# safes/RayTracing-Weekend

Hardware: AMD Instinct MI355X
Metric: Msamples/s, Cornell box 1920x1080 4096spp (higher is better)
Workload: dtype f32

## Files before the change

raytracing_weekend_amd/csrc/rtw_device.h:

```cpp
#pragma once
#include <hip/hip_runtime.h>
#include <stdint.h>

#include "../../include/rtw.h"

#define RTW_DEV __device__ __forceinline__

#define RTW_MATH_FN RTW_DEV
#include "rtw_math.h"
#include "rtw_scene.h"

#ifndef RTW_SHORT_FORMS
#define RTW_SHORT_FORMS 1
#endif

namespace rtwdev {

struct v3 { float x, y, z; };

RTW_DEV v3 V(float x, float y, float z) { v3 r; r.x = x; r.y = y; r.z = z; return r; }
RTW_DEV v3 vadd(v3 a, v3 b) { return V(a.x + b.x, a.y + b.y, a.z + b.z); }
RTW_DEV v3 vsub(v3 a, v3 b) { return V(a.x - b.x, a.y - b.y, a.z - b.z); }
RTW_DEV v3 vmul(v3 a, v3 b) { return V(a.x * b.x, a.y * b.y, a.z * b.z); }
RTW_DEV v3 vscale(v3 a, float s) { return V(a.x * s, a.y * s, a.z * s); }
RTW_DEV v3 vneg(v3 a) { return V(-a.x, -a.y, -a.z); }
RTW_DEV float fma_(float a, float b, float c) { return __builtin_fmaf(a, b, c); }
RTW_DEV v3 vfma(v3 a, float s, v3 b) { return V(fma_(a.x, s, b.x), fma_(a.y, s, b.y), fma_(a.z, s, b.z)); }
RTW_DEV float dot3(v3 a, v3 b) { return fma_(a.z, b.z, fma_(a.y, b.y, a.x * b.x)); }
RTW_DEV v3 cross3(v3 a, v3 b) {
    return V(fma_(a.y, b.z, -(a.z * b.y)), fma_(a.z, b.x, -(a.x * b.z)), fma_(a.x, b.y, -(a.y * b.x)));
}
struct MathHw {
    static RTW_DEV float rcp(float x) { return __builtin_amdgcn_rcpf(x); }
    static RTW_DEV float rsq(float x) { return __builtin_amdgcn_rsqf(x); }
    static RTW_DEV float fma(float a, float b, float c) { return __builtin_fmaf(a, b, c); }
    static RTW_DEV bool all(bool ok) { return __builtin_amdgcn_ballot_w64(!ok) == 0ull; }
};
RTW_DEV float rcp_(float x) { return RTW_SHORT_FORMS ? rtwmath::rcp<MathHw>(x) : 1.0f / x; }
RTW_DEV float sqrt_(float x) { return RTW_SHORT_FORMS ? rtwmath::sqrt<MathHw>(x) : __builtin_sqrtf(x); }
RTW_DEV float sqrt_inside_(float x) { return RTW_SHORT_FORMS ? rtwmath::sqrt_inside<MathHw>(x) : __builtin_sqrtf(x); }
RTW_DEV v3 normalize3(v3 a) {
    const float s = dot3(a, a);
    const float inv = RTW_SHORT_FORMS ? rtwmath::rcp_sqrt<MathHw>(s) : 1.0f / __builtin_sqrtf(s);
    return vscale(a, inv);
}
RTW_DEV float length3(v3 a) { return sqrt_(dot3(a, a)); }
// ... 228 lines not shown
    }
};

typedef uint32_t u32x4 __attribute__((ext_vector_type(4)));
typedef float f32x4 __attribute__((ext_vector_type(4)));

struct DScene {
    const rtw_prim* __restrict__ prims;
    const rtw_xform* __restrict__ xforms;
    const HitRec* __restrict__ hitrec;
    const rtw_light* __restrict__ lights;
    const u32x4* __restrict__ nodes;
    const u32x4* __restrict__ leaves;
    const u32x4* __restrict__ wnodes;
    const int32_t* __restrict__ order;
    const BruteGroup* __restrict__ groups;
    const BruteRec* __restrict__ recs;
    const rtw_texture* __restrict__ texs;
    const uint32_t* __restrict__ texdata;
    const u32x4* __restrict__ walk;
    int32_t n_prims, n_vol, n_tree, n_lights, sky_light, use_bvh, has_motion, n_groups;
    int32_t n_generic;
    int32_t n_walk_words;
    int32_t n_lds_nodes, stack_depth, has_tex, noise_lds_data;
    int32_t n_lds_leaves, stack_wide;
    int32_t n_nodes;
    int32_t estimator;
    float ray_tmin, probe_eps;
    const rtw_light* __restrict__ clights;
    float bmin[3], bmax[3];
    rtw_camera cam;
    rtw_pdf pdf;
    int32_t cam_type;
};

RTW_DEV bool is_volume(int type) { return type == RTW_PRIM_VOLUME_BOX || type == RTW_PRIM_VOLUME_SPHERE; }

#define RTW_CONST __attribute__((address_space(4)))
template <class T>
RTW_DEV const RTW_CONST T* as_const(const T* p) { return (const RTW_CONST T*)(uint64_t)p; }

RTW_DEV rtw_prim load_prim(const DScene& sc, int i) {
    const RTW_CONST u32x4* q = (const RTW_CONST u32x4*)(uint64_t)(sc.prims + i);
    u32x4 a = q[0], b = q[1], c = q[2], d = q[3];
    rtw_prim r;
    r.type = (int)a.x; r.material = (int)a.y; r.xform = (int)a.z; r.flip = (int)a.w;
    r.p[0] = __uint_as_float(b.x); r.p[1] = __uint_as_float(b.y); r.p[2] = __uint_as_float(b.z); r.p[3] = __uint_as_float(b.w);
    r.p[4] = __uint_as_float(c.x); r.p[5] = __uint_as_float(c.y); r.p[6] = __uint_as_float(c.z); r.p[7] = __uint_as_float(c.w);
    r.p[8] = __uint_as_float(d.x); r.p[9] = __uint_as_float(d.y); r.p[10] = __uint_as_float(d.z); r.p[11] = __uint_as_float(d.w);
    return r;
}
struct M34 { float m[12]; };
RTW_DEV M34 load_m34(const float* p) {
    const RTW_CONST f32x4* q = (const RTW_CONST f32x4*)(uint64_t)p;
    f32x4 a = q[0], b = q[1], c = q[2];
    M34 r;
    r.m[0] = a.x; r.m[1] = a.y; r.m[2] = a.z; r.m[3] = a.w;
    r.m[4] = b.x; r.m[5] = b.y; r.m[6] = b.z; r.m[7] = b.w;
    r.m[8] = c.x; r.m[9] = c.y; r.m[10] = c.z; r.m[11] = c.w;
    return r;
}
RTW_DEV M34 load_xf_m(const DScene& sc, int i) { return load_m34(sc.xforms[i].m); }
RTW_DEV M34 load_xf_inv(const DScene& sc, int i) { return load_m34(sc.xforms[i].inv); }
RTW_DEV int load_i32(const int32_t* p) { return *as_const(p); }
typedef uint32_t u32x8 __attribute__((ext_vector_type(8)));
RTW_DEV BruteGroup load_group(const DScene& sc, int i) {
// ... 433 lines not shown
            RTW_RECT_LOOP(G.n_rx, oo.x, inv.x, oo.y, dd.y, oo.z, dd.z)
            RTW_RECT_LOOP(G.n_ry, oo.y, inv.y, oo.x, dd.x, oo.z, dd.z)
            RTW_RECT_LOOP(G.n_rz, oo.z, inv.z, oo.x, dd.x, oo.y, dd.y)
#undef RTW_RECT_LOOP
        }
        for (int i = 0; i < G.n_sph; i++) {
            const BruteRec Rn = load_rec(sc, ++ri);
            float t = 0.f;
            const bool hit = sphere_roots(oo, dd, V(R.a, R.b, R.c), R.d, tmin, RTW_FLT_MAX, t);
            RTW_TAKE(hit, t, R.prim)
            R = Rn;
        }
    }
#undef RTW_TAKE
    if (!GENERIC || (ANY_HIT && best_prim >= 0)) return;
    for (int k = 0; k < sc.n_generic; k++) {
        const int pi = load_i32(sc.order + sc.n_vol + k);
        const rtw_prim pr = load_prim(sc, pi);
        v3 po, pd, mt;
        object_ray(sc, pr, o, d, ray_time, po, pd, mt);
        float t;
        if (prim_test(pr, po, pd, V(0.f, 0.f, 0.f), tmin, RTW_FLT_MAX, gather_time, g, t)) {
            if (t < best_t || (!ANY_HIT && t == best_t && best_prim >= 0 && !best_is_vol && pi < best_prim)) {
                best_t = t; best_prim = pi; best_is_vol = false;
                if (ANY_HIT) return;
            }
        }
    }
}

struct WalkRec { u32x4 q0, q1; };
RTW_DEV bool in_range(float a, uint32_t lo, uint32_t hi) { return __builtin_amdgcn_fmed3f(a, __uint_as_float(lo), __uint_as_float(hi)) == a; }

template <bool ANY_HIT>
RTW_DEV void walk_lds(const u32x4* __restrict__ w, const int n_groups, const v3 o, const v3 d, const float tmin, const float tmax, float& best_t, int& best_prim) {
    uint32_t key_hi = __float_as_uint(tmax), key_lo = 0u;
    const u32x4* xf = w + 2 * n_groups;
    const u32x4* r = w + 5 * n_groups;
    WalkRec A, B;
    A.q0 = r[0]; A.q1 = r[1];
#define RTW_RECT_TEST(R_, OK_, IK_, OA_, DA_, OB_, DB_)                                              \
    {                                                                                                \
        const float t = (__uint_as_float(R_.q1.x) - (OK_)) * (IK_);                                  \
        const float a = fma_(t, (DA_), (OA_));                                                       \
        const float b = fma_(t, (DB_), (OB_));                                                       \
        const bool hit = (t >= tmin) & in_range(a, R_.q0.x, R_.q0.y) & in_range(b, R_.q0.z, R_.q0.w); \
        if (ANY_HIT) {                                                                               \
            key_lo = (hit & (t < tmax)) ? 1u : key_lo;                                               \
        } else {                                                                                     \
            const unsigned long long key = ((unsigned long long)__float_as_uint(t) << 32) | R_.q1.y; \
            const bool take = hit & (key < (((unsigned long long)key_hi << 32) | key_lo));           \
            key_hi = take ? __float_as_uint(t) : key_hi;                                             \
            key_lo = take ? R_.q1.y : key_lo;                                                        \
        }                                                                                            \
    }
#define RTW_REC_LIST(N_, TEST_)                                                                      \
    {                                                                                                \
        int n_ = (N_);                                                                               \
        for (; n_ >= 2; n_ -= 2) {                                                                   \
            B.q0 = r[2]; B.q1 = r[3];                                                                \
            TEST_(A)                                                                                 \
            A.q0 = r[4]; A.q1 = r[5];                                                                \
            TEST_(B)                                                                                 \
            r += 4;                                                                                  \
        }                                                                                            \
        if (n_ > 0) {                                                                                \
            B.q0 = r[2]; B.q1 = r[3];                                                                \
            TEST_(A)                                                                                 \
            A = B;                                                                                   \
            r += 2;                                                                                  \
        }                                                                                            \
    }
    for (int gi = 0; gi < n_groups; gi++) {
        const u32x4 g0 = w[2 * gi], g1 = w[2 * gi + 1];
        const int g_xform = (int)__builtin_amdgcn_readfirstlane(g0.x);
        const int n_rx = (int)__builtin_amdgcn_readfirstlane(g0.z), n_ry = (int)__builtin_amdgcn_readfirstlane(g0.w);
        const int n_rz = (int)__builtin_amdgcn_readfirstlane(g1.x), n_sph = (int)__builtin_amdgcn_readfirstlane(g1.y);
        v3 oo = o, dd = d;
        if (g_xform != 0) {
            const u32x4 r0 = xf[3 * gi], r1 = xf[3 * gi + 1], r2 = xf[3 * gi + 2];
            float m[12];
            m[0] = __uint_as_float(r0.x); m[1] = __uint_as_float(r0.y); m[2] = __uint_as_float(r0.z); m[3] = __uint_as_float(r0.w);
            m[4] = __uint_as_float(r1.x); m[5] = __uint_as_float(r1.y); m[6] = __uint_as_float(r1.z); m[7] = __uint_as_float(r1.w);
            m[8] = __uint_as_float(r2.x); m[9] = __uint_as_float(r2.y); m[10] = __uint_as_float(r2.z); m[11] = __uint_as_float(r2.w);
            oo = xf_point(m, o);
            dd = xf_vector(m, d);
        }
        if (n_rx + n_ry + n_rz > 0) {
            const v3 inv = recip3(dd);
#define RTW_TEST_X(R_) RTW_RECT_TEST(R_, oo.x, inv.x, oo.y, dd.y, oo.z, dd.z)
#define RTW_TEST_Y(R_) RTW_RECT_TEST(R_, oo.y, inv.y, oo.x, dd.x, oo.z, dd.z)
#define RTW_TEST_Z(R_) RTW_RECT_TEST(R_, oo.z, inv.z, oo.x, dd.x, oo.y, dd.y)
            RTW_REC_LIST(n_rx, RTW_TEST_X)
            RTW_REC_LIST(n_ry, RTW_TEST_Y)
            RTW_REC_LIST(n_rz, RTW_TEST_Z)
#undef RTW_TEST_X
#undef RTW_TEST_Y
#undef RTW_TEST_Z
        }
#define RTW_TEST_SPH(R_)                                                                             \
        {                                                                                            \
            float t = 0.f;                                                                           \
            const bool hit = sphere_roots(oo, dd, V(__uint_as_float(R_.q0.x), __uint_as_float(R_.q0.y), __uint_as_float(R_.q0.z)), \
                                          __uint_as_float(R_.q0.w), tmin, RTW_FLT_MAX, t);           \
            if (ANY_HIT) {                                                                           \
                key_lo = (hit & (t < tmax)) ? 1u : key_lo;                                           \
            } else {                                                                                 \
                const unsigned long long key = ((unsigned long long)__float_as_uint(t) << 32) | R_.q1.y; \
                const bool take = hit & (key < (((unsigned long long)key_hi << 32) | key_lo));       \
                key_hi = take ? __float_as_uint(t) : key_hi;                                         \
// ... 352 lines not shown
```

raytracing_weekend_amd/csrc/rtw_hip.hip:

```cpp
#include <hip/hip_runtime.h>

#include <algorithm>
#include <cmath>
#include <cstdio>
#include <cstdlib>
#include <cstring>
#include <condition_variable>
#include <exception>
#include <mutex>
#include <new>
#include <stdexcept>
#include <string>
#include <thread>
#include <vector>

#include "../../include/rtw.h"
#include "rtw_bvh.h"
#include "rtw_scene.h"
#include "rtw_device.h"
#include "rtw_plan.h"
#include "rtw_kernels.h"
#include "rtw_guides.h"
#include "rtw_adaptive.h"
#ifndef RTW_SPLIT_BUILD
// ... 358 lines not shown
    if (c->d_scene) (void)hipFree(c->d_scene);
    if (c->stream) (void)hipStreamDestroy(c->stream);
    delete c;
    return RTW_OK;
}

int upload_prepared(rtw_ctx* c, const PreparedScene& ps) {
    test_fault("upload");
    HIP_TRY(c, hipSetDevice(c->device));
    HIP_TRY(c, hipStreamSynchronize(c->stream));
    if (c->d_scene) { (void)hipFree(c->d_scene); c->d_scene = nullptr; }
    c->has_scene = false;
    HIP_TRY(c, hipMalloc(&c->d_scene, ps.image.size()));
    HIP_TRY(c, hipMemcpy(c->d_scene, ps.image.data(), ps.image.size(), hipMemcpyHostToDevice));
    const char* d = (const char*)c->d_scene;
    const SceneScalars& v = ps.sc;
    const SceneFacts& f = ps.info.facts;
    DScene sc{};
    sc.prims = (const rtw_prim*)(d + ps.off[ST_PRIMS]);
    sc.xforms = (const rtw_xform*)(d + ps.off[ST_XFORMS]);
    sc.hitrec = (const HitRec*)(d + ps.off[ST_HITREC]);
    sc.lights = (const rtw_light*)(d + ps.off[ST_LIGHTS]);
    sc.clights = (const rtw_light*)(d + ps.off[ST_CLIGHTS]);
    sc.nodes = (const u32x4*)(d + ps.off[ST_NODES]);
    sc.wnodes = (const u32x4*)(d + ps.off[ST_WNODES]);
    sc.leaves = (const u32x4*)(d + ps.off[ST_LEAVES]);
    sc.order = (const int32_t*)(d + ps.off[ST_ORDER]);
    sc.groups = (const BruteGroup*)(d + ps.off[ST_GROUPS]);
    sc.recs = (const BruteRec*)(d + ps.off[ST_RECS]);
    sc.texs = (const rtw_texture*)(d + ps.off[ST_TEXS]);
    sc.texdata = (const uint32_t*)(d + ps.off[ST_TEXDATA]);
    sc.walk = (const u32x4*)(d + ps.off[ST_WALK]);
    sc.n_prims = v.n_prims; sc.n_tree = v.n_tree; sc.n_lights = v.n_lights; sc.sky_light = v.sky_light; sc.has_motion = v.has_motion;
    sc.n_groups = v.n_groups; sc.n_generic = v.n_generic; sc.n_walk_words = v.n_walk_words; sc.n_lds_nodes = v.n_lds_nodes; sc.has_tex = v.has_tex;
    sc.noise_lds_data = v.noise_lds_data; sc.n_lds_leaves = v.n_lds_leaves; sc.cam_type = v.cam_type;
    sc.use_bvh = f.use_bvh ? 1 : 0; sc.n_vol = f.n_vol; sc.stack_depth = f.stack_depth; sc.stack_wide = f.stack_wide ? 1 : 0; sc.n_nodes = (int32_t)f.n_tree_nodes;
    sc.estimator = RTW_EST_REFERENCE; sc.ray_tmin = 1e-6f; sc.probe_eps = 500 * 1.0e-7f;
    for (int a = 0; a < 3; a++) { sc.bmin[a] = v.bmin[a]; sc.bmax[a] = v.bmax[a]; }
    sc.cam = v.cam;
    sc.pdf = v.pdf;
    c->sc = sc;
    c->info = ps.info;
    c->has_scene = true;
    return RTW_OK;
}

int impl_upload_scene(rtw_ctx* c, const void* blob, size_t bytes) {
    if (!c) return RTW_ERR_INVALID_ARG;
    if (!c->kids.empty()) c->has_scene = false;
    PreparedScene ps;
    std::string err;
    const int prc = prepare_scene(blob, bytes, read_tuning(), ps, err);
    if (prc) return fail(c, prc, err);
    if (c->kids.empty()) return upload_prepared(c, ps);
    for (rtw_ctx* k : c->kids) {
        const int rc = upload_prepared(k, ps);
        if (rc) return fail(c, rc, k->err);
    }
    c->has_scene = true;
    return RTW_OK;
}

int check_render_args(rtw_ctx* c, const rtw_params* P) {
    if (!c->has_scene) return fail(c, RTW_ERR_NO_SCENE, "rtw_render before rtw_upload_scene");
    if (!P) return fail(c, RTW_ERR_INVALID_ARG, "null params");
    if (P->width <= 0 || P->height <= 0 || P->spp <= 0 || P->max_depth < 0 || P->row0 < 0 || P->row1 > P->height || P->row0 > P->row1)
        return fail(c, RTW_ERR_INVALID_ARG, "bad render params");
// ... 974 lines not shown
```

raytracing_weekend_amd/csrc/rtw_kernels.h:

```cpp
#pragma once
#include "rtw_device.h"
#include "rtw_plan.h"

namespace rtwk {
using namespace rtwdev;

#ifndef RTW_MIN_WAVES
#define RTW_MIN_WAVES 1
#endif
#ifdef RTW_SUBPHASE_TIMERS
constexpr int kSubRows = 16, kSubWaves = 8192;
__device__ unsigned long long g_sub_cyc[kSubWaves][kSubRows];
RTW_DEV constexpr int rtw_sub_id(const char* n) {
    return n[0] != 's' || n[1] != 'a' ? 0 : n[3] == 'h' ? 1 : n[3] == 'l' && n[4] == 'a' ? 2 : n[3] == 'l' ? 3 : n[3] == 'm' ? 4 : n[3] == 'd' ? 5 : n[3] == 'i' ? 6 : n[3] == 'n' ? 7 : 0;
}
RTW_DEV void rtw_sub_stamp(int id) {
    const unsigned long long t_in = __builtin_amdgcn_s_memtime();
    if ((threadIdx.x & 63u) == 0u) {
        unsigned long long* row = g_sub_cyc[(blockIdx.x * (blockDim.x >> 6) + (threadIdx.x >> 6)) % kSubWaves];
        const unsigned long long open_id = row[14], t0 = row[15];
        if (t0 != 0ull) row[open_id] += t_in - t0;
        row[14] = (unsigned long long)id;
        __builtin_amdgcn_s_waitcnt(0);
        row[15] = __builtin_amdgcn_s_memtime();
// ... 1045 lines not shown
                bool alive = false;
                uint32_t nee_prev = (p.gk & kNeePrev) ? 1u : 0u;
                for (uint32_t it = 0; it < A.n_iter; it++) {
                    float t;
                    int prim;
                    traverse<Rng<KIND>, false, false>(A.sc, p.o, p.d, A.sc.ray_tmin, 1.e27f, p.ray_time, gt, g, tm, t, prim);
                    v3 so, sd, att, radiance;
                    Nee nee;
                    const int ev = shade_a<KIND, TEX>(A.sc, g, p.o, p.d, gt, t, prim, so, sd, att, radiance, nee, noise_lds, nee_prev);
                    n_seg++;
                    if (nee.has) {
                        float st;
                        int sprim;
                        traverse<Rng<KIND>, true, false>(A.sc, so, nee.dir, nee.tmin, nee.tmax, 0.0f, gt, g, tm, st, sprim);
                        n_shadow++;
                        if (sprim < 0) radiance = vadd(radiance, nee.rad);
                    }
                    alive = shade_b<KIND>(depth, A.max_depth, g, ev, so, sd, att, radiance, p.o, p.d, p.T, p.L, TEX == 2 && A.sc.estimator == RTW_EST_MIXTURE);
                    depth++;
                    if (!alive) break;
                    p.ray_time = (KIND == RTW_RNG_TEA_LCG || A.sc.has_motion) ? g.ray_time(depth) : 0.0f;
                }
                p.a = g.a; p.b = g.b;
                p.gk = (p.gk & ~kNeePrev) | (nee_prev ? kNeePrev : 0u);
                if (alive) keep = true;
                else finish_path(A, path_id_of<KIND>(A, p), p.L);
            }
        }
        compact_store(A, s_cursor, keep, p);
    }
    cursor_publish(A, s_cursor, n_seg, n_shadow, RTW_K_BOUNCE);
}

RTW_DEV uint32_t order_lookup(const KArgs& A, uint32_t gi) {
    const uint32_t n_groups = (A.npix + 63u) / 64u;
    const uint32_t c2 = A.order_counts[0], c1 = A.order_counts[1];
    const uint32_t idx = gi < c2 ? gi : (gi < c2 + c1 ? n_groups + (gi - c2) : 2u * n_groups + (gi - c2 - c1));
    return __builtin_amdgcn_readfirstlane(A.order[idx]);
}

template <bool WALK>
__global__ void __launch_bounds__(kBlock) k_classify(const KArgs A, uint32_t* __restrict__ order, uint32_t* __restrict__ counters, uint32_t n_groups) {
    __shared__ u32x4 s_walk[WALK ? kWalkMaxWords : 1];
    if (WALK) {
        for (uint32_t i = threadIdx.x; i < (uint32_t)A.sc.n_walk_words; i += kBlock) s_walk[i] = A.sc.walk[i];
        __syncthreads();
    }
    const uint32_t lane = threadIdx.x & 63u;
    const uint32_t waves = gridDim.x * (kBlock / 64u);
    for (uint32_t g = blockIdx.x * (kBlock / 64u) + (threadIdx.x >> 6); g < n_groups; g += waves) {
        const uint32_t p_local = g * 64u + lane;
        bool may = false, specular = false, inside = false;
        if (p_local < A.npix) {
            const uint32_t yl = fastdiv(p_local, A.divw_m, A.divw_s1, A.divw_s2);
            const uint32_t x = p_local - yl * A.width, y = A.row0 + yl * A.row_stride;
            inside = (int32_t)x >= A.cull_x0 && (int32_t)x < A.cull_x1 && (int32_t)y >= A.cull_y0 && (int32_t)y < A.cull_y1;
            const rtw_camera& cam = A.sc.cam;
            if (A.sc.cam_type != RTW_CAM_PERSPECTIVE || cam.lens_radius != 0.0f) {
                may = true;
            } else {
                const float s = ((float)x + 0.5f) / (float)A.width, t = ((float)y + 0.5f) / (float)A.height;
                const v3 o = ld3(cam.origin);
                const v3 d = vsub(vfma(ld3(cam.vertical), t, vfma(ld3(cam.horizontal), s, ld3(cam.lower_left))), o);
                may = may_hit_scene(A.sc, o, d);
                if (WALK && may) {
                    float th;
                    int prim;
                    walk_lds<false>(s_walk, A.sc.n_groups, o, d, A.sc.ray_tmin, 1.e27f, th, prim);
                    if (prim >= 0) {
                        const int mt = A.sc.hitrec[prim].mat_type;
                        specular = mt == RTW_MAT_METAL || mt == RTW_MAT_DIELECTRIC;
                    }
                }
            }
        }
        if (__ballot(inside) == 0ull) continue;
        const bool any = __ballot(may) != 0ull;
        const uint32_t n_spec = (uint32_t)__popcll(__ballot(specular));
        if (lane == 0) {
            const uint32_t cls = !any ? 0u : (n_spec >= 16u ? 2u : 1u);
            order[(2u - cls) * n_groups + atomicAdd(&counters[2u - cls], 1u)] = g;
        }
    }
}

#if defined(RTW_PHASE_TIMERS)
#define RTW_MARK(name) { const unsigned long long now_ = __builtin_amdgcn_s_memtime(); ph_cyc[ph_cur] += now_ - ph_t0; ph_t0 = now_; ph_cur = rtw_phase_id(name); }
RTW_DEV constexpr int rtw_phase_id(const char* n) { return n[0] == 'r' && n[2] == 'f' ? 0 : n[0] == 'r' ? 1 : n[0] == 'w' && n[5] == 'r' ? 2 : n[0] == 's' && n[6] == 'a' ? 3 : n[0] == 'w' ? 4 : 5; }
#else
#define RTW_MARK(name) asm volatile("; MARK " name)
#endif
#ifndef RTW_PATH_WAVES
#define RTW_PATH_WAVES 5
#endif
#ifndef RTW_PATH_COLD_WAVES
#define RTW_PATH_COLD_WAVES RTW_MIN_WAVES
#endif
template <int KIND, int TEX, int MEDIA5 = 0, int LIST = 0>
__global__ void __launch_bounds__(kBlock, TEX ? (MEDIA5 ? 5 : RTW_PATH_COLD_WAVES) : RTW_PATH_WAVES) k_path(const KArgs A) {
    RTW_NOISE_SHARED
    __shared__ u32x4 s_hitrec[kPathMaxPrims * 6];
    const uint32_t tid = threadIdx.x;
    const uint32_t* noise_lds = stage_noise<(TEX != 0)>(A.sc, s_noise);
    {
        const u32x4* src = (const u32x4*)A.sc.hitrec;
        for (uint32_t i = tid; i < (uint32_t)A.sc.n_prims * 6u; i += kBlock) s_hitrec[i] = src[i];
    }
    __shared__ float s_usum[3][kBlock];
    __shared__ PathConsts s_pc;
    if (tid == 0) {
        for (int q = 0; q < 3; q++) {
            s_pc.cam_o[q] = A.sc.cam.origin[q]; s_pc.cam_ll[q] = A.sc.cam.lower_left[q];
            s_pc.cam_h[q] = A.sc.cam.horizontal[q]; s_pc.cam_v[q] = A.sc.cam.vertical[q];
        }
        for (int q = 0; q < 5; q++) s_pc.rect[q] = A.sc.pdf.rect[q];
        int gen = A.sc.pdf.gen;
        if (gen == RTW_PDF_MIXTURE || gen == RTW_PDF_MIXTURE_BIAS) gen = A.sc.pdf.p1_gen;
        s_pc.gen = gen;
        if (A.sc.n_lights > 0) {
            for (int q = 0; q < 3; q++) { s_pc.lnrm[q] = A.sc.lights[0].normal[q]; s_pc.lemi[q] = A.sc.lights[0].emission[q]; }
            s_pc.larea = A.sc.lights[0].area;
        }
        s_pc.npix = LIST ? A.order[0] : A.npix; s_pc.width = A.width; s_pc.row0 = A.row0; s_pc.row_stride = A.row_stride;
        s_pc.divs_m = A.divs_m; s_pc.divs_s1 = A.divs_s1; s_pc.divs_s2 = A.divs_s2; s_pc.spp = A.spp;
        s_pc.bs_lo = (uint32_t)(uint64_t)A.blocksum; s_pc.bs_hi = (uint32_t)((uint64_t)A.blocksum >> 32);
        s_pc.unit_shift = (A.unit_sums && !LIST) ? 3u : 0u; s_pc.list_lo = LIST ? (uint32_t)(uint64_t)(A.order + 1) : 0u;
        s_pc.n_jobs = A.n_jobs; s_pc.n_ranges = A.n_ranges; s_pc.units_per_job = A.units_per_job; s_pc.unit_blocks = A.unit_blocks;
        s_pc.n_blocks_pass = A.n_blocks_pass; s_pc.block0 = A.block0; s_pc.divw_m = A.divw_m; s_pc.divw_s1 = A.divw_s1; s_pc.divw_s2 = A.divw_s2;
        s_pc.q_lo = (uint32_t)(uint64_t)A.queue; s_pc.q_hi = (uint32_t)((uint64_t)A.queue >> 32); s_pc.list_hi = LIST ? (uint32_t)((uint64_t)(A.order + 1) >> 32) : 0u;
    }
    const PathConsts* pc_cam = TEX ? nullptr : &s_pc;
    __shared__ u32x4 s_walk[TEX ? 1 : kWalkMaxWords];
    if (!TEX) for (uint32_t i = tid; i < (uint32_t)A.sc.n_walk_words; i += kBlock) s_walk[i] = A.sc.walk[i];
    __syncthreads();
    const uint32_t lane = tid & 63u;
    uint32_t u_next = 0, u_end = 0, job_g = 0, job_b = 0;
    bool exhausted = false;
    bool need = true;
    uint32_t pxy = 0, blk = 0, blk_end = 0, s_cur = 0;
    v3 usum = V(0.f, 0.f, 0.f);
    bool alive = false;
    uint32_t depth = 0, rng_a = 0;
    uint32_t gk = 0, rng_b = 0, nee_prev = 0;
    float ray_time = 0.f;
    v3 o = V(0.f, 0.f, 0.f), d = o, T = o, L = o;
    uint32_t n_seg = 0, n_shadow = 0;
#ifdef RTW_PHASE_TIMERS
    unsigned long long ph_cyc[6] = {0, 0, 0, 0, 0, 0}, ph_t0 = __builtin_amdgcn_s_memtime();
    int ph_cur = 0;
#endif
    for (;;) {
        RTW_MARK("refill");
        unsigned long long need_mask = __ballot(need);
        while (need_mask != 0ull && !exhausted) {
            const PathConsts* kc = &s_pc;
            if (u_next >= u_end) {
                uint32_t q = 0;
                if (lane == 0) q = atomicAdd((uint32_t*)(((uint64_t)kc->q_hi << 32) | kc->q_lo), 1u);
                q = __builtin_amdgcn_readfirstlane(q);
                if (q >= (uint32_t)__builtin_amdgcn_readfirstlane((int)kc->n_jobs)) { exhausted = true; break; }
                const uint32_t n_ranges = (uint32_t)__builtin_amdgcn_readfirstlane((int)kc->n_ranges), upj = (uint32_t)__builtin_amdgcn_readfirstlane((int)kc->units_per_job);
                const uint32_t gi = q / n_ranges;
                job_g = LIST ? gi : order_lookup(A, gi);
                job_b = (q - gi * n_ranges) * upj;
                u_next = 0; u_end = 64u * upj;
                continue;
            }
            const uint32_t avail = u_end - u_next;
            const uint32_t rank = __builtin_amdgcn_mbcnt_hi((uint32_t)(need_mask >> 32), __builtin_amdgcn_mbcnt_lo((uint32_t)need_mask, 0u));
            if (need && rank < avail) {
                const uint32_t ub = kc->unit_blocks, nbp = kc->n_blocks_pass;
                const uint32_t u = u_next + rank;
                const uint32_t b = (job_b + (u >> 6)) * ub;
                const uint32_t p_local = job_g * 64u + (u & 63u);
                if (p_local < kc->npix && b < nbp) {
                    need = false;
                    blk = b;
                    blk_end = min(b + ub, nbp);
                    uint32_t pix = p_local;
                    if (LIST) {
                        pix = ((const uint32_t*)(((uint64_t)kc->list_hi << 32) | kc->list_lo))[p_local];
                        s_usum[0][tid] = __uint_as_float(p_local);
                    }
                    const uint32_t yl = fastdiv(pix, kc->divw_m, kc->divw_s1, kc->divw_s2);
                    pxy = (pix - yl * kc->width) | ((kc->row0 + yl * kc->row_stride) << 16);
                    s_cur = (kc->block0 + b) * kSumBlock;
                    usum = V(0.f, 0.f, 0.f);
                    alive = false;
                }
            }
            u_next += min((uint32_t)__popcll(need_mask), avail);
            need_mask = __ballot(need);
        }
        if (__ballot(!need) == 0ull) break;
        RTW_MARK("regen");
        const bool busy = !need;
        const uint32_t px = pxy & 0xffffu, py = pxy >> 16;
        Rng<KIND> g;
        if (busy && !alive) {
            Path p;
            raygen<KIND, !TEX>(A, px, py, A.sample0 + s_cur, 0u, p, g, pc_cam);
            o = p.o; d = p.d; T = p.T; L = p.L; rng_a = p.a;
            if (TEX) { ray_time = p.ray_time; gk = p.gk; rng_b = p.b; nee_prev = 0; }
            depth = 0; alive = true;
        }
        if (busy) {
            const uint32_t pixel = A.width * py + px;
            if (KIND == RTW_RNG_TEA_LCG) g.init(A.seed, 0, 0, rng_a, rng_b);
            else g.init(A.seed, pixel, A.sample0 + s_cur, rng_a, A.sample0 + s_cur);
        }
        RTW_MARK("walk_r");
        const float gt = TEX ? gather_time_of(A, gk) : 0.0f;
        float th = 1.e27f;
        int prim = -1;
        const bool walk = busy && (depth > 0u || may_hit_scene(A.sc, o, d));
        if (__ballot(walk) != 0ull) {
            if (busy) {
                if (TEX) traverse_brute<Rng<KIND>, false, false>(A.sc, o, d, A.sc.ray_tmin, 1.e27f, ray_time, gt, g, th, prim);
                else walk_lds<false>(s_walk, A.sc.n_groups, o, d, A.sc.ray_tmin, 1.e27f, th, prim);
            }
        }
        RTW_MARK("shade_a");
#ifdef RTW_SUBPHASE_TIMERS
        rtw_sub_stamp(8);
#endif
        if (busy) {
            v3 so, sd, att, radiance;
            Nee nee;
            const int ev = shade_a<KIND, TEX>(A.sc, g, o, d, gt, th, prim, so, sd, att, radiance, nee, noise_lds, nee_prev, s_hitrec, &s_pc);
            n_seg++;
#ifdef RTW_SUBPHASE_TIMERS
            rtw_sub_stamp(0);
#endif
            RTW_MARK("walk_s");
            if (nee.has) {
                float st;
                int sprim;
                if (TEX) traverse_brute<Rng<KIND>, true, false>(A.sc, so, nee.dir, nee.tmin, nee.tmax, 0.0f, gt, g, st, sprim);
                else walk_lds<true>(s_walk, A.sc.n_groups, so, nee.dir, nee.tmin, nee.tmax, st, sprim);
                n_shadow++;
                if (sprim < 0) radiance = vadd(radiance, nee.rad);
            }
            RTW_MARK("shade_b");
            alive = shade_b<KIND>(depth, A.max_depth, g, ev, so, sd, att, radiance, o, d, T, L, TEX == 2 && A.sc.estimator == RTW_EST_MIXTURE);
            depth++;
            rng_a = g.a;
            if (alive) {
                if (TEX) {
                    ray_time = (KIND == RTW_RNG_TEA_LCG || A.sc.has_motion) ? g.ray_time(depth) : 0.0f;
                    rng_b = g.b;
                }
            } else {
                usum = vadd(usum, V((L.x == L.x) ? L.x : 0.f, (L.y == L.y) ? L.y : 0.f, (L.z == L.z) ? L.z : 0.f));
                s_cur++;
                if ((s_cur % kSumBlock) == 0u || s_cur >= A.spp) {
                    const PathConsts* kc = &s_pc;
                    const uint32_t c_row0 = kc->row0, c_stride = kc->row_stride, c_width = kc->width, c_npix = kc->npix;
                    const uint32_t yl_ = c_stride > 1 ? fastdiv(py - c_row0, kc->divs_m, kc->divs_s1, kc->divs_s2) : py - c_row0;
                    const uint32_t pix = LIST ? __float_as_uint(s_usum[0][tid]) : yl_ * c_width + px;
                    const uint32_t b_done = blk;
                    blk++;
                    need = blk >= blk_end || s_cur >= A.spp;
                    float4* const bsum_base = (float4*)(((uint64_t)kc->bs_hi << 32) | kc->bs_lo);
                    const uint32_t ush = kc->unit_shift;
                    v3 prev = V(0.f, 0.f, 0.f);
                    if (ush != 0u && (b_done % kSumUnitBlocks) != 0u) prev = V(s_usum[0][tid], s_usum[1][tid], s_usum[2][tid]);
                    const v3 u = vadd(prev, usum);
                    if (ush == 0u || need || (blk % kSumUnitBlocks) == 0u) bsum_base[(size_t)(b_done >> ush) * c_npix + pix] = make_float4(u.x, u.y, u.z, 0.f);
                    else { s_usum[0][tid] = u.x; s_usum[1][tid] = u.y; s_usum[2][tid] = u.z; }
                    usum = V(0.f, 0.f, 0.f);
                }
            }
// ... 157 lines not shown
```

raytracing_weekend_amd/csrc/rtw_scene.h:

```cpp
#pragma once
#include <stdint.h>

#include <algorithm>
#include <cmath>
#include <cstdio>
#include <cstring>
#include <string>
#include <vector>

#include "../../include/rtw.h"
#include "rtw_bvh.h"
#include "rtw_plan.h"

namespace rtwdev {

enum { HK_CONST_NORMAL = 0, HK_SPHERE = 1, HK_MOVING_SPHERE = 2, HK_SPHERE_XFORM = 3 };
struct HitRec {
    int32_t mat_type;
    int32_t bsdf_eval;
    float param;
    int32_t kind;
    float r, g, b;
    float inv_r;
    float nx, ny, nz;
    int32_t xform;
    float ux, uy, uz; int32_t tex_dyn;
    float vx, vy, vz; int32_t listed;
    float wx, wy, wz, pad2;
};

struct BruteGroup {
    int32_t xform;
    int32_t first;
    int32_t n_rx, n_ry, n_rz, n_sph;
    int32_t pad0, pad1;
};
struct BruteRec {
    float a, b, c, d, e;
    int32_t prim;
    int32_t pad0, pad1;
};

constexpr int kWalkMaxWords = 400;

}

namespace rtwk {

enum SceneTable { ST_PRIMS, ST_XFORMS, ST_HITREC, ST_LIGHTS, ST_CLIGHTS, ST_NODES, ST_WNODES, ST_LEAVES, ST_ORDER, ST_GROUPS, ST_RECS, ST_TEXS, ST_TEXDATA,
                  ST_WALK, ST_COUNT };

struct SceneScalars {
    int32_t n_prims, n_tree, n_lights, sky_light, has_motion, n_groups, n_generic, n_walk_words;
    int32_t n_lds_nodes, has_tex, noise_lds_data, n_lds_leaves, cam_type;
    float bmin[3], bmax[3];
    rtw_camera cam;
    rtw_pdf pdf;
};
struct SceneInfo {
    SceneFacts facts;
    size_t lds_bytes;
    bool cull_ok;
    float cull_bmin[3], cull_bmax[3];
};
struct PreparedScene {
    std::vector<char> image;
    size_t off[ST_COUNT];
    SceneScalars sc;
    SceneInfo info;
};

namespace scene_detail {
using namespace rtwdev;

struct Tables {
    rtw_scene_header h;
    std::vector<rtw_prim> prims;
    std::vector<rtw_xform> xforms;
    std::vector<rtw_material> mats;
    std::vector<rtw_texture> texs;
    std::vector<rtw_light> lights;
    std::vector<uint32_t> texdata;
};

inline int fail(std::string& err, const char* msg, int code = RTW_ERR_BAD_SCENE) {
    err = msg;
    return code;
// ... 125 lines not shown
    return r;
}

inline void build_lists(const Tables& s, bool use_bvh, std::vector<int32_t>& order, int& n_vol, std::vector<BruteGroup>& groups, std::vector<BruteRec>& recs) {
    const size_t n = s.prims.size();
    for (size_t i = 0; i < n; i++) if (rtwbvh::is_volume(s.prims[i].type)) order.push_back((int32_t)i);
    n_vol = (int)order.size();
    if (use_bvh) return;
    for (size_t i = 0; i < n; i++) if (s.prims[i].type == RTW_PRIM_MOVING_SPHERE) order.push_back((int32_t)i);
    auto listable = [](int t) { return !rtwbvh::is_volume(t) && t != RTW_PRIM_MOVING_SPHERE; };
    for (size_t first = 0; first < n; first++) {
        const int xf = s.prims[first].xform;
        if (!listable(s.prims[first].type) || std::any_of(groups.begin(), groups.end(), [&](const BruteGroup& g) { return g.xform == xf; })) continue;
        BruteGroup g{};
        g.xform = xf;
        g.first = (int32_t)recs.size();
        const int kinds[4] = {RTW_PRIM_RECT_X, RTW_PRIM_RECT_Y, RTW_PRIM_RECT_Z, RTW_PRIM_SPHERE};
        int32_t* counts[4] = {&g.n_rx, &g.n_ry, &g.n_rz, &g.n_sph};
        for (int k = 0; k < 4; k++)
            for (size_t i = first; i < n; i++) {
                const rtw_prim& p = s.prims[i];
                if (p.type != kinds[k] || p.xform != xf) continue;
                BruteRec r{};
                r.a = p.p[0]; r.b = p.p[1]; r.c = p.p[2]; r.d = p.p[3];
                if (k < 3) r.e = p.p[4];
                r.prim = (int32_t)i;
                recs.push_back(r);
                (*counts[k])++;
            }
        groups.push_back(g);
    }
}

inline std::vector<uint32_t> walk_image(const Tables& s, const std::vector<BruteGroup>& groups, const std::vector<BruteRec>& recs) {
    static_assert(sizeof(BruteGroup) == 32 && sizeof(BruteRec) == 32, "walk image layout");
    const size_t ng = groups.size(), words = 5 * ng + 2 * recs.size() + 4;
    if (ng == 0 || words > (size_t)kWalkMaxWords) return {};
    std::vector<uint32_t> walk(words * 4, 0u);
    memcpy(walk.data(), groups.data(), ng * sizeof(BruteGroup));
    for (size_t g = 0; g < ng; g++) memcpy(&walk[(2 * ng + 3 * g) * 4], s.xforms[groups[g].xform].inv, 12 * sizeof(float));
    for (size_t i = 0; i < recs.size(); i++) {
        memcpy(&walk[(5 * ng + 2 * i) * 4], &recs[i], sizeof(BruteRec));
        walk[(5 * ng + 2 * i) * 4 + 5] = (uint32_t)recs[i].prim + 1u;
    }
    return walk;
}

inline void pad_wave_nodes(std::vector<rtwbvh::WNode>& wq4, float big) {
    const float pad = 1.0e-4f + big * (1.0f / 524288.0f);
    for (rtwbvh::WNode& w : wq4)
        for (int k = 0; k < 4; k++)
            if (w.ref[k] != rtwbvh::kQ4Empty)
                for (int a = 0; a < 3; a++) { w.box[k][a] -= pad; w.box[k][3 + a] += pad; }
}

template <class T>
void stage(PreparedScene& out, SceneTable t, const std::vector<T>& v, size_t min_elems = 0, size_t extra = 0) {
    out.off[t] = out.image.size();
    out.image.resize((out.off[t] + (std::max(v.size(), min_elems) + extra) * sizeof(T) + 255u) & ~size_t(255), 0);
    if (!v.empty()) memcpy(out.image.data() + out.off[t], v.data(), v.size() * sizeof(T));
}

}

inline int prepare_scene(const void* blob, size_t bytes, const Tuning& tune, PreparedScene& out, std::string& err) {
    using namespace scene_detail;
    Tables s;
    if (const int rc = parse_scene(blob, bytes, s, err)) return rc;
    const rtw_scene_header& h = s.h;
    out = PreparedScene{};
    SceneScalars& sc = out.sc;
    SceneFacts& facts = out.info.facts;

    std::vector<rtw_light> clights;
    std::vector<uint8_t> listed;
    match_lights(s, clights, listed);
    std::vector<HitRec> hitrec(h.n_prims);
    bool dyn_tex = false;
    rtwbvh::Box all;
    float big = 1.0f;
    for (uint32_t i = 0; i < h.n_prims; i++) {
        hitrec[i] = bake_hitrec(s, i, listed[i] != 0);
        dyn_tex = dyn_tex || (hitrec[i].kind >> 8) != 0;
        if (s.prims[i].type == RTW_PRIM_MOVING_SPHERE) sc.has_motion = 1;
        const rtwbvh::Box wb = rtwbvh::world_bounds(s.prims[i], s.xforms[s.prims[i].xform]);
        all.add(wb);
        for (int a = 0; a < 3; a++) big = std::max(big, std::max(std::fabs(wb.mn[a]), std::fabs(wb.mx[a])));
    }
    for (int a = 0; a < 3; a++) big = std::max(big, std::fabs(h.camera.origin[a]) + std::fabs(h.camera.lens_radius));

    facts.use_bvh = (int)h.n_prims > tune.brute_max;
    std::vector<int32_t> order;
    std::vector<BruteGroup> groups;
    std::vector<BruteRec> recs;
    build_lists(s, facts.use_bvh, order, facts.n_vol, groups, recs);
    sc.n_generic = (int)order.size() - facts.n_vol;
    const std::vector<uint32_t> walk = !facts.use_bvh && sc.n_generic == 0 ? walk_image(s, groups, recs) : std::vector<uint32_t>();
    rtwbvh::Bvh bvh;
    if (facts.use_bvh) {
        bvh = rtwbvh::build_bvh(s.prims.data(), h.n_prims, s.xforms.data());
        if (bvh.stack_need > 95) return fail(err, "tree deeper than the LDS traversal stack", RTW_ERR_UNSUPPORTED);
        if (bvh.max_exp > 60) return fail(err, "scene extent beyond 1e20", RTW_ERR_UNSUPPORTED);
        pad_wave_nodes(bvh.wq4, big);
        facts.stack_depth = bvh.stack_need + 2;
        facts.stack_wide = (std::max(bvh.q4.size(), (size_t)bvh.n_slots) << 2) >= 0x7ff0u;
        facts.n_tree_nodes = bvh.q4.size();
        facts.n_tree_leaves = bvh.n_slots;
        out.info.lds_bytes = tree_lds_layout(facts.n_tree_nodes, facts.n_tree_leaves, facts.stack_depth, facts.stack_wide, kBlock, tune.lds_kb * 1024, sc.n_lds_nodes, sc.n_lds_leaves);
        if (tune.verbose) fprintf(stderr, "[rtw] tree (SAH bins %d, collapse %d, sample-walk cost %.3f): %zu nodes, %zu leaf records, stack %d x %d bit; LDS %zu B: %d nodes, %d leaf records\n", bvh.bins, bvh.collapse_kind, bvh.cost,
                                  bvh.q4.size(), (size_t)bvh.n_slots, facts.stack_depth, facts.stack_wide ? 32 : 16, out.info.lds_bytes, sc.n_lds_nodes, sc.n_lds_leaves);
    }

    stage(out, ST_PRIMS, s.prims);
    stage(out, ST_XFORMS, s.xforms);
    stage(out, ST_HITREC, hitrec);
    stage(out, ST_LIGHTS, s.lights, 1);
    stage(out, ST_CLIGHTS, clights, 1);
    stage(out, ST_NODES, bvh.q4, 1);
    stage(out, ST_WNODES, bvh.wq4, 1);
    stage(out, ST_LEAVES, bvh.leaves, 1);
    stage(out, ST_ORDER, order, 1);
    stage(out, ST_GROUPS, groups, 1);
    stage(out, ST_RECS, recs, 0, 1);
    stage(out, ST_TEXS, s.texs, 1);
    stage(out, ST_TEXDATA, s.texdata, 1);
    stage(out, ST_WALK, walk, 1);

    sc.n_prims = (int)h.n_prims;
    sc.n_tree = (int)bvh.prim_order.size();
    sc.n_lights = (int)h.n_lights;
    sc.sky_light = h.sky_light;
    sc.n_groups = (int)groups.size();
    sc.n_walk_words = (int32_t)(walk.size() / 4);
    sc.has_tex = (dyn_tex || facts.n_vol > 0 || sc.n_generic > 0 || h.camera_type != RTW_CAM_PERSPECTIVE || h.camera.lens_radius != 0.0f) ? 1 : 0;
    sc.noise_lds_data = -1;
    for (uint32_t i = 0; i < h.n_prims && sc.noise_lds_data < 0; i++) {
        int ti = s.mats[s.prims[i].material].texture;
        if (ti < 0) continue;
        if (s.texs[ti].type == RTW_TEX_CHECKER) ti = s.texs[s.texs[ti].odd].type == RTW_TEX_NOISE ? s.texs[ti].odd : s.texs[ti].even;
        if (s.texs[ti].type == RTW_TEX_NOISE) sc.noise_lds_data = (int32_t)s.texs[ti].data;
    }
    {
        float diag = 0.f;
        for (int a = 0; a < 3; a++) diag += (all.mx[a] - all.mn[a]) * (all.mx[a] - all.mn[a]);
        const float pad = 0.01f * std::sqrt(diag) + 1.0f;
        for (int a = 0; a < 3; a++) { sc.bmin[a] = all.mn[a] - pad; sc.bmax[a] = all.mx[a] + pad; }
    }
    sc.cam = h.camera;
    sc.pdf = h.pdf;
    sc.cam_type = h.camera_type;
    out.info.cull_ok = cull_bounds(s.prims.data(), h.n_prims, s.xforms.data(), h.camera, out.info.cull_bmin, out.info.cull_bmax);
    return RTW_OK;
}

}
```

Before: 18140.

## Pack walk group headers into compact LDS words and skip scene-bounds ballot for near jobs

Adds a packed header layout in which each brute-force walk group's xform flag and four record counts fit in one 32-bit word, four groups per LDS vector. The traversal reads these headers with one LDS load per four groups and scalarizes them, replacing two u32x4 loads per group. It also skips the may_hit_scene ballot for pixel jobs classified as near by the order lookup, walking unconditionally there. Costs: more header-decode ALU work, extra shared memory, and fallback paths for scenes whose counts don't fit.

```diff
diff --git a/raytracing_weekend_amd/csrc/rtw_device.h b/raytracing_weekend_amd/csrc/rtw_device.h
--- a/raytracing_weekend_amd/csrc/rtw_device.h
+++ b/raytracing_weekend_amd/csrc/rtw_device.h
@@ -12,6 +12,9 @@
 
 #ifndef RTW_SHORT_FORMS
 #define RTW_SHORT_FORMS 1
+#endif
+#ifndef RTW_WALK_PACKED
+#define RTW_WALK_PACKED 1
 #endif
 
 namespace rtwdev {
@@ -306,6 +309,7 @@
     rtw_camera cam;
     rtw_pdf pdf;
     int32_t cam_type;
+    int32_t n_walk_hdr;
 };
 
 RTW_DEV bool is_volume(int type) { return type == RTW_PRIM_VOLUME_BOX || type == RTW_PRIM_VOLUME_SPHERE; }
@@ -805,13 +809,22 @@
 struct WalkRec { u32x4 q0, q1; };
 RTW_DEV bool in_range(float a, uint32_t lo, uint32_t hi) { return __builtin_amdgcn_fmed3f(a, __uint_as_float(lo), __uint_as_float(hi)) == a; }
 
-template <bool ANY_HIT>
-RTW_DEV void walk_lds(const u32x4* __restrict__ w, const int n_groups, const v3 o, const v3 d, const float tmin, const float tmax, float& best_t, int& best_prim) {
+template <bool ANY_HIT, bool HDR>
+RTW_DEV void walk_lds(const u32x4* __restrict__ w, const u32x4* __restrict__ hdr, const int n_groups, const v3 o, const v3 d, const float tmin, const float tmax,
+                      float& best_t, int& best_prim) {
     uint32_t key_hi = __float_as_uint(tmax), key_lo = 0u;
     const u32x4* xf = w + 2 * n_groups;
     const u32x4* r = w + 5 * n_groups;
     WalkRec A, B;
     A.q0 = r[0]; A.q1 = r[1];
+    uint32_t h0 = 0u, h1 = 0u, h2 = 0u, h3 = 0u;
+    if (HDR) {
+        u32x4 hw = hdr[0];
+        asm volatile("" : "+v"(A.q0), "+v"(A.q1), "+v"(hw));
+        h0 = __builtin_amdgcn_readfirstlane(hw.x); h1 = __builtin_amdgcn_readfirstlane(hw.y);
+        h2 = __builtin_amdgcn_readfirstlane(hw.z); h3 = __builtin_amdgcn_readfirstlane(hw.w);
+    }
+    const bool packed = HDR && (h0 & kWalkHdrValid) != 0u;
 #define RTW_RECT_TEST(R_, OK_, IK_, OA_, DA_, OB_, DB_)                                              \
     {                                                                                                \
         const float t = (__uint_as_float(R_.q1.x) - (OK_)) * (IK_);                                  \
@@ -845,10 +858,24 @@
         }                                                                                            \
     }
     for (int gi = 0; gi < n_groups; gi++) {
-        const u32x4 g0 = w[2 * gi], g1 = w[2 * gi + 1];
-        const int g_xform = (int)__builtin_amdgcn_readfirstlane(g0.x);
-        const int n_rx = (int)__builtin_amdgcn_readfirstlane(g0.z), n_ry = (int)__builtin_amdgcn_readfirstlane(g0.w);
-        const int n_rz = (int)__builtin_amdgcn_readfirstlane(g1.x), n_sph = (int)__builtin_amdgcn_readfirstlane(g1.y);
+        int g_xform, n_rx, n_ry, n_rz, n_sph;
+        if (packed) {
+            const uint32_t m = (uint32_t)kWalkHdrMaxCount;
+            g_xform = (int)(h0 & 1u);
+            n_rx = (int)((h0 >> 1) & m); n_ry = (int)((h0 >> (1 + kWalkHdrCountBits)) & m);
+            n_rz = (int)((h0 >> (1 + 2 * kWalkHdrCountBits)) & m); n_sph = (int)((h0 >> (1 + 3 * kWalkHdrCountBits)) & m);
+            h0 = h1; h1 = h2; h2 = h3;
+            if ((gi & 3) == 3 && gi + 1 < n_groups) {
+                const u32x4 hw = hdr[(gi + 1) >> 2];
+                h0 = __builtin_amdgcn_readfirstlane(hw.x); h1 = __builtin_amdgcn_readfirstlane(hw.y);
+                h2 = __builtin_amdgcn_readfirstlane(hw.z); h3 = __builtin_amdgcn_readfirstlane(hw.w);
+            }
+        } else {
+            const u32x4 g0 = w[2 * gi], g1 = w[2 * gi + 1];
+            g_xform = (int)__builtin_amdgcn_readfirstlane(g0.x);
+            n_rx = (int)__builtin_amdgcn_readfirstlane(g0.z); n_ry = (int)__builtin_amdgcn_readfirstlane(g0.w);
+            n_rz = (int)__builtin_amdgcn_readfirstlane(g1.x); n_sph = (int)__builtin_amdgcn_readfirstlane(g1.y);
+        }
         v3 oo = o, dd = d;
         if (g_xform != 0) {
             const u32x4 r0 = xf[3 * gi], r1 = xf[3 * gi + 1], r2 = xf[3 * gi + 2];
diff --git a/raytracing_weekend_amd/csrc/rtw_hip.hip b/raytracing_weekend_amd/csrc/rtw_hip.hip
--- a/raytracing_weekend_amd/csrc/rtw_hip.hip
+++ b/raytracing_weekend_amd/csrc/rtw_hip.hip
@@ -414,7 +414,7 @@
     sc.texdata = (const uint32_t*)(d + ps.off[ST_TEXDATA]);
     sc.walk = (const u32x4*)(d + ps.off[ST_WALK]);
     sc.n_prims = v.n_prims; sc.n_tree = v.n_tree; sc.n_lights = v.n_lights; sc.sky_light = v.sky_light; sc.has_motion = v.has_motion;
-    sc.n_groups = v.n_groups; sc.n_generic = v.n_generic; sc.n_walk_words = v.n_walk_words; sc.n_lds_nodes = v.n_lds_nodes; sc.has_tex = v.has_tex;
+    sc.n_groups = v.n_groups; sc.n_generic = v.n_generic; sc.n_walk_words = v.n_walk_words; sc.n_walk_hdr = v.n_walk_hdr; sc.n_lds_nodes = v.n_lds_nodes; sc.has_tex = v.has_tex;
     sc.noise_lds_data = v.noise_lds_data; sc.n_lds_leaves = v.n_lds_leaves; sc.cam_type = v.cam_type;
     sc.use_bvh = f.use_bvh ? 1 : 0; sc.n_vol = f.n_vol; sc.stack_depth = f.stack_depth; sc.stack_wide = f.stack_wide ? 1 : 0; sc.n_nodes = (int32_t)f.n_tree_nodes;
     sc.estimator = RTW_EST_REFERENCE; sc.ray_tmin = 1e-6f; sc.probe_eps = 500 * 1.0e-7f;
diff --git a/raytracing_weekend_amd/csrc/rtw_kernels.h b/raytracing_weekend_amd/csrc/rtw_kernels.h
--- a/raytracing_weekend_amd/csrc/rtw_kernels.h
+++ b/raytracing_weekend_amd/csrc/rtw_kernels.h
@@ -1101,9 +1101,10 @@
     cursor_publish(A, s_cursor, n_seg, n_shadow, RTW_K_BOUNCE);
 }
 
-RTW_DEV uint32_t order_lookup(const KArgs& A, uint32_t gi) {
+RTW_DEV uint32_t order_lookup(const KArgs& A, uint32_t gi, bool& far) {
     const uint32_t n_groups = (A.npix + 63u) / 64u;
     const uint32_t c2 = A.order_counts[0], c1 = A.order_counts[1];
+    far = gi >= c2 + c1;
     const uint32_t idx = gi < c2 ? gi : (gi < c2 + c1 ? n_groups + (gi - c2) : 2u * n_groups + (gi - c2 - c1));
     return __builtin_amdgcn_readfirstlane(A.order[idx]);
 }
@@ -1135,7 +1136,7 @@
                 if (WALK && may) {
                     float th;
                     int prim;
-                    walk_lds<false>(s_walk, A.sc.n_groups, o, d, A.sc.ray_tmin, 1.e27f, th, prim);
+                    walk_lds<false, false>(s_walk, nullptr, A.sc.n_groups, o, d, A.sc.ray_tmin, 1.e27f, th, prim);
                     if (prim >= 0) {
                         const int mt = A.sc.hitrec[prim].mat_type;
                         specular = mt == RTW_MAT_METAL || mt == RTW_MAT_DIELECTRIC;
@@ -1161,6 +1162,9 @@
 #endif
 #ifndef RTW_PATH_WAVES
 #define RTW_PATH_WAVES 5
+#endif
+#ifndef RTW_FAR_ZONE
+#define RTW_FAR_ZONE 1
 #endif
 #ifndef RTW_PATH_COLD_WAVES
 #define RTW_PATH_COLD_WAVES RTW_MIN_WAVES
@@ -1200,11 +1204,16 @@
     }
     const PathConsts* pc_cam = TEX ? nullptr : &s_pc;
     __shared__ u32x4 s_walk[TEX ? 1 : kWalkMaxWords];
-    if (!TEX) for (uint32_t i = tid; i < (uint32_t)A.sc.n_walk_words; i += kBlock) s_walk[i] = A.sc.walk[i];
+    __shared__ u32x4 s_whdr[TEX ? 1 : kWalkHdrMaxWords];
+    if (!TEX) {
+        for (uint32_t i = tid; i < (uint32_t)A.sc.n_walk_words; i += kBlock) s_walk[i] = A.sc.walk[i];
+        if (tid < (uint32_t)kWalkHdrMaxWords) s_whdr[tid] = tid < (uint32_t)A.sc.n_walk_hdr ? A.sc.walk[(uint32_t)A.sc.n_walk_words + tid] : u32x4{0u, 0u, 0u, 0u};
+    }
     __syncthreads();
     const uint32_t lane = tid & 63u;
     uint32_t u_next = 0, u_end = 0, job_g = 0, job_b = 0;
     bool exhausted = false;
+    bool far = !RTW_FAR_ZONE || TEX || LIST;
     bool need = true;
     uint32_t pxy = 0, blk = 0, blk_end = 0, s_cur = 0;
     v3 usum = V(0.f, 0.f, 0.f);
@@ -1230,7 +1239,9 @@
                 if (q >= (uint32_t)__builtin_amdgcn_readfirstlane((int)kc->n_jobs)) { exhausted = true; break; }
                 const uint32_t n_ranges = (uint32_t)__builtin_amdgcn_readfirstlane((int)kc->n_ranges), upj = (uint32_t)__builtin_amdgcn_readfirstlane((int)kc->units_per_job);
                 const uint32_t gi = q / n_ranges;
-                job_g = LIST ? gi : order_lookup(A, gi);
+                bool far_job = false;
+                job_g = LIST ? gi : order_lookup(A, gi, far_job);
+                far = far || far_job;
                 job_b = (q - gi * n_ranges) * upj;
                 u_next = 0; u_end = 64u * upj;
                 continue;
@@ -1282,11 +1293,12 @@
         const float gt = TEX ? gather_time_of(A, gk) : 0.0f;
         float th = 1.e27f;
         int prim = -1;
-        const bool walk = busy && (depth > 0u || may_hit_scene(A.sc, o, d));
-        if (__ballot(walk) != 0ull) {
+        bool any_walk = true;
+        if (far) any_walk = __ballot(busy && (depth > 0u || may_hit_scene(A.sc, o, d))) != 0ull;
+        if (any_walk) {
             if (busy) {
                 if (TEX) traverse_brute<Rng<KIND>, false, false>(A.sc, o, d, A.sc.ray_tmin, 1.e27f, ray_time, gt, g, th, prim);
-                else walk_lds<false>(s_walk, A.sc.n_groups, o, d, A.sc.ray_tmin, 1.e27f, th, prim);
+                else walk_lds<false, RTW_WALK_PACKED != 0>(s_walk, s_whdr, A.sc.n_groups, o, d, A.sc.ray_tmin, 1.e27f, th, prim);
             }
         }
         RTW_MARK("shade_a");
@@ -1306,7 +1318,7 @@
                 float st;
                 int sprim;
                 if (TEX) traverse_brute<Rng<KIND>, true, false>(A.sc, so, nee.dir, nee.tmin, nee.tmax, 0.0f, gt, g, st, sprim);
-                else walk_lds<true>(s_walk, A.sc.n_groups, so, nee.dir, nee.tmin, nee.tmax, st, sprim);
+                else walk_lds<true, RTW_WALK_PACKED != 0>(s_walk, s_whdr, A.sc.n_groups, so, nee.dir, nee.tmin, nee.tmax, st, sprim);
                 n_shadow++;
                 if (sprim < 0) radiance = vadd(radiance, nee.rad);
             }
diff --git a/raytracing_weekend_amd/csrc/rtw_scene.h b/raytracing_weekend_amd/csrc/rtw_scene.h
--- a/raytracing_weekend_amd/csrc/rtw_scene.h
+++ b/raytracing_weekend_amd/csrc/rtw_scene.h
@@ -43,6 +43,18 @@
 
 constexpr int kWalkMaxWords = 400;
 
+constexpr int kWalkHdrMaxWords = 8, kWalkHdrCountBits = 7, kWalkHdrMaxCount = (1 << kWalkHdrCountBits) - 1;
+constexpr uint32_t kWalkHdrValid = 0x80000000u;
+inline bool pack_walk_hdr(const BruteGroup& g, uint32_t& word) {
+    const int32_t n[4] = {g.n_rx, g.n_ry, g.n_rz, g.n_sph};
+    word = kWalkHdrValid | (g.xform != 0 ? 1u : 0u);
+    for (int k = 0; k < 4; k++) {
+        if (n[k] < 0 || n[k] > kWalkHdrMaxCount) return false;
+        word |= (uint32_t)n[k] << (1 + kWalkHdrCountBits * k);
+    }
+    return true;
+}
+
 }
 
 namespace rtwk {
@@ -53,6 +65,7 @@
 struct SceneScalars {
     int32_t n_prims, n_tree, n_lights, sky_light, has_motion, n_groups, n_generic, n_walk_words;
     int32_t n_lds_nodes, has_tex, noise_lds_data, n_lds_leaves, cam_type;
+    int32_t n_walk_hdr;
     float bmin[3], bmax[3];
     rtw_camera cam;
     rtw_pdf pdf;
@@ -244,11 +257,17 @@
     }
 }
 
-inline std::vector<uint32_t> walk_image(const Tables& s, const std::vector<BruteGroup>& groups, const std::vector<BruteRec>& recs) {
+inline std::vector<uint32_t> walk_image(const Tables& s, const std::vector<BruteGroup>& groups, const std::vector<BruteRec>& recs, size_t& hdr_words) {
     static_assert(sizeof(BruteGroup) == 32 && sizeof(BruteRec) == 32, "walk image layout");
     const size_t ng = groups.size(), words = 5 * ng + 2 * recs.size() + 4;
+    hdr_words = 0;
     if (ng == 0 || words > (size_t)kWalkMaxWords) return {};
-    std::vector<uint32_t> walk(words * 4, 0u);
+    std::vector<uint32_t> hdr((ng + 3) / 4 * 4, 0u);
+    bool packs = hdr.size() / 4 <= (size_t)kWalkHdrMaxWords && words + hdr.size() / 4 <= (size_t)kWalkMaxWords;
+    for (size_t g = 0; g < ng && packs; g++) packs = pack_walk_hdr(groups[g], hdr[g]);
+    if (packs) hdr_words = hdr.size() / 4;
+    std::vector<uint32_t> walk((words + hdr_words) * 4, 0u);
+    if (packs) memcpy(&walk[words * 4], hdr.data(), hdr.size() * sizeof(uint32_t));
     memcpy(walk.data(), groups.data(), ng * sizeof(BruteGroup));
     for (size_t g = 0; g < ng; g++) memcpy(&walk[(2 * ng + 3 * g) * 4], s.xforms[groups[g].xform].inv, 12 * sizeof(float));
     for (size_t i = 0; i < recs.size(); i++) {
@@ -307,7 +326,8 @@
     std::vector<BruteRec> recs;
     build_lists(s, facts.use_bvh, order, facts.n_vol, groups, recs);
     sc.n_generic = (int)order.size() - facts.n_vol;
-    const std::vector<uint32_t> walk = !facts.use_bvh && sc.n_generic == 0 ? walk_image(s, groups, recs) : std::vector<uint32_t>();
+    size_t walk_hdr = 0;
+    const std::vector<uint32_t> walk = !facts.use_bvh && sc.n_generic == 0 ? walk_image(s, groups, recs, walk_hdr) : std::vector<uint32_t>();
     rtwbvh::Bvh bvh;
     if (facts.use_bvh) {
         bvh = rtwbvh::build_bvh(s.prims.data(), h.n_prims, s.xforms.data());
@@ -343,7 +363,8 @@
     sc.n_lights = (int)h.n_lights;
     sc.sky_light = h.sky_light;
     sc.n_groups = (int)groups.size();
-    sc.n_walk_words = (int32_t)(walk.size() / 4);
+    sc.n_walk_hdr = (int32_t)walk_hdr;
+    sc.n_walk_words = (int32_t)(walk.size() / 4 - walk_hdr);
     sc.has_tex = (dyn_tex || facts.n_vol > 0 || sc.n_generic > 0 || h.camera_type != RTW_CAM_PERSPECTIVE || h.camera.lens_radius != 0.0f) ? 1 : 0;
     sc.noise_lds_data = -1;
     for (uint32_t i = 0; i < h.n_prims && sc.noise_lds_data < 0; i++) {
```

New measurement: 18280 (median of 6 runs). Within noise of the previous version (+0.8%).
